# YukeWang96/QGTC_PPoPP22

Measured on AMD Instinct MI355X. Metric: effective bit-GEMM TOPS (2*M*K*N/t), 1-bit A x 1-bit X, M=K=4096, N=64, higher is better.
Workload: dtype fp4 (E2M1 codes of bit planes on MFMA, exact f32 sums); 1 GPU; bitMM2Bit 4096x4096x64 a=1 w=1 ob=1 (BASELINE.json configs[1], 2_7c shape); inputs=seeded Bernoulli(0.5) adjacency, uniform w-bit features, packed, resident in HBM, parallelism=replica-per-GPU x1, no data-path collective, engine=auto, issue=eager

## Files before the change

__graft_entry__.py:

```python
from __future__ import annotations

import os
import sys

ROOT = os.path.dirname(os.path.abspath(__file__))
if ROOT not in sys.path:
    sys.path.insert(0, ROOT)


def build() -> None:
    from qgtc_ppopp22_amd import _build

    paths = _build.build_all()
    from oracle import qgtc_oracle

    paths["oracle"] = qgtc_oracle.build()
    import qgtc_ppopp22_amd

    ext = qgtc_ppopp22_amd.load_ext()
    assert ext.abi_version() == 11
    import ctypes

    lib = ctypes.CDLL(qgtc_ppopp22_amd.lib_path())
    for sym in ("qgtc_abi_version", "qgtc_strerror", "qgtc_last_hip_error", "qgtc_rows_words",
                "qgtc_cols_words", "qgtc_val2bit", "qgtc_bit2val", "qgtc_bitmm2bit", "qgtc_bitmm2int",
                "qgtc_bitmm2bit_profile", "qgtc_tile_counters", "qgtc_bitmm_batched", "qgtc_pack_edges",
                "qgtc_i8gemm", "qgtc_i8gemm_profile", "qgtc_occupancy_words", "qgtc_tile_occupancy",
                "qgtc_tile_occupancy_batched", "qgtc_tile_occupancy_decide", "qgtc_pack_edge_list",
                "qgtc_gcn_layer_batched", "qgtc_gcn_chain_batched", "qgtc_last_batched_violation",
                "qgtc_val2bit_batched", "qgtc_epoch_pool_layout", "qgtc_epoch_plan_fill", "qgtc_expand_weights", "qgtc_chain_transform",
                "qgtc_chain_aggregate", "qgtc_chain_words", "qgtc_weight_codes_words", "qgtc_chain_from_cols",
                "qgtc_adj_tiles_words", "qgtc_adj_tiles_from_rows", "qgtc_load_batches", "qgtc_load_work_words", "qgtc_bitmm_route", "qgtc_bitmm_batched_route",
                "qgtc_tiled_work_words", "qgtc_tiled_count", "qgtc_tiled_fill", "qgtc_tiledmm2bit", "qgtc_tiledmm2int",
                "qgtc_tiled_colindex_work_words", "qgtc_tiled_colindex", "qgtc_tiledmm2bit_t", "qgtc_tiledmm2int_t",
                "qgtc_tiled_degrees", "qgtc_tiledmm2bit_scaled", "qgtc_tiledmm2int_scaled", "qgtc_tiledmm2bit_t_scaled", "qgtc_tiledmm2int_t_scaled",
                "qgtc_tiledmm_f32", "qgtc_tiledmm_f32_t", "qgtc_tiledmm_f32_src", "qgtc_tiledmm_f32_t_src", "qgtc_tiled_inv_sqrt_degree",
                "qgtc_tiledmax_f32", "qgtc_tiledmax_f32_t", "qgtc_tiledsel_f32", "qgtc_tiledsel_f32_t",
                "qgtc_tiledatt_f32", "qgtc_tiledatt_f32_t", "qgtc_tiledatt_grad_f32", "qgtc_tiledatt_grad_f32_t", "qgtc_rowdot_f32",
                "qgtc_edge_kept", "qgtc_tiledmm_f32_drop", "qgtc_tiledmm_f32_t_drop", "qgtc_tiledmax_f32_drop", "qgtc_tiledmax_f32_t_drop",
                "qgtc_tiledatt_f32_drop", "qgtc_tiledatt_f32_t_drop", "qgtc_tiledatt_grad_f32_drop", "qgtc_tiledatt_grad_f32_t_drop",
                "qgtc_node_bitmap", "qgtc_tiled_inv_degree", "qgtc_tiledmm_f32_nodes", "qgtc_tiledmm_f32_t_nodes", "qgtc_tiledmax_f32_nodes",
                "qgtc_tiledmax_f32_t_nodes", "qgtc_tiledatt_f32_nodes", "qgtc_tiledatt_f32_t_nodes", "qgtc_tiledatt_grad_f32_nodes",
                "qgtc_tiledatt_grad_f32_t_nodes", "qgtc_tiled_value_index", "qgtc_tiled_edge_slots", "qgtc_tiled_edge_endpoints",
                "qgtc_tiledmm_f32_edge", "qgtc_tiledmm_f32_t_edge", "qgtc_tiled_sddmm_f32", "qgtc_reorder_work_words", "qgtc_reorder_nodes"):
        getattr(lib, sym)
    print("[build] ok:", paths)


def smoke() -> None:
    import numpy as np
    import torch

    assert torch.cuda.is_available(), "smoke() needs a GPU"
    import QGTC
    from oracle.qgtc_oracle import Oracle

    O = Oracle()
    rng = np.random.default_rng(3)
    n, F, H, b = 300, 64, 64, 2
    A = (rng.random((n, n)) < 0.02).astype(np.float32)
    X = rng.normal(size=(n, F)).astype(np.float32)
    W = np.ones((F, H), dtype=np.float32)

    dA, dX, dW = (torch.from_numpy(t).cuda() for t in (A, X, W))
    bit_A = QGTC.val2bit(dA, 1, False, False)
    bit_X = QGTC.val2bit(dX, b, False, False)
    bit_W = QGTC.val2bit(dW, b, True, False)
# ... 82 lines not shown
```

include/qgtc.h:

```cpp
#ifndef QGTC_H
#define QGTC_H

#include <stddef.h>
#include <stdint.h>

#ifdef __cplusplus
extern "C" {
#endif

#define QGTC_ABI_VERSION 11

enum {
    QGTC_OK = 0,
    QGTC_EINVAL = 1,
    QGTC_ESIZE = 2,
    QGTC_EALIGN = 3,
    QGTC_EHIP = 4,
    QGTC_ENODEVICE = 5
};

#define QGTC_OUT_COLS 0x1u
#define QGTC_NO_ZERO_SKIP 0x2u
#define QGTC_ZERO_JUMP 0x4u
#define QGTC_ENGINE_MFMA 0x8u
// ... 46 lines not shown
int qgtc_tile_occupancy(const uint32_t *X, size_t x_words, int M, int K, int bit1, uint64_t *occ,
                        size_t occ_words, void *stream);

int qgtc_tile_occupancy_batched(qgtc_problem *problems, int count, int max_M, int max_K, int bit1,
                                float max_fraction, uint64_t *stats, void *stream);

int qgtc_tile_occupancy_decide(qgtc_problem *problems, int count, float max_fraction, uint64_t *stats,
                               void *stream);

int qgtc_bitmm_batched(const qgtc_problem *problems, int count, int max_M, int max_K, int max_N,
                       int bit1, int bit2, int output_bit, int mode, unsigned flags,
                       void *stream);

int qgtc_gcn_layer_batched(const qgtc_problem *stage1, const qgtc_problem *stage2, int count, int max_M, int max_K1,
                           int max_K2, int max_N, int x_bits, int w_bits, int t_bits, int a_bits, int output_bit,
                           int mode, unsigned flags, void *stream);

int qgtc_gcn_chain_batched(const qgtc_problem *stage_a, const qgtc_problem *stage_xw, int count, int max_M, int max_K,
                           int max_N1, int max_N2, int a_bits, int t_bits, int act_bits, int w_bits, int out_bits,
                           int out_mode, unsigned flags, void *stream);

const char *qgtc_bitmm_route(int M, int K, int N, int bit1, int bit2, int output_bit, int mode, unsigned flags);
const char *qgtc_bitmm_batched_route(int max_M, int max_K, int max_N, int bit1, int bit2, int output_bit, int mode, unsigned flags);

int qgtc_pack_edges(const int64_t *cells, const int32_t *counts, size_t n_cells, int H, int W,
                    int nbits, uint32_t *out, size_t out_words, void *stream);

int qgtc_pack_edge_list(const int64_t *src, const int64_t *dst, size_t n_edges, int H, int W, uint32_t *out,
                        size_t out_words, uint32_t *scratch, size_t scratch_words, int *bad_index, void *stream);

int qgtc_i8gemm(const int8_t *A, const int8_t *Bt, int M, int K, int N, float *C, size_t c_elems,
                void *stream);
int qgtc_i8gemm_profile(const int8_t *A, const int8_t *Bt, int M, int K, int N, float *C,
                        size_t c_elems, int reps, float *elapsed_ms, void *stream);

enum { QGTC_VIOL_NONE = 0, QGTC_VIOL_M = 1, QGTC_VIOL_K = 2, QGTC_VIOL_N = 3, QGTC_VIOL_POINTER = 4, QGTC_VIOL_CHAINING = 5 };
int qgtc_last_batched_violation(int *problem, int *field, void *stream);

#define QGTC_MAX_PACK_JOBS 8
typedef struct qgtc_pack_job {
    const float *x;
    uint32_t *out;
    uint64_t out_words;
    int32_t H, W, nbits, col_major, output_layer;
    int32_t reserved;
} qgtc_pack_job;
// ... 238 lines not shown
```

qgtc_ppopp22_amd/csrc/launch_common.hip.h:

```cpp
#pragma once

#include <algorithm>
#include <atomic>

int qgtc_launch_mfma(const qgtc_problem &pr, int a, int w, int ob, int mode, hipStream_t st);
int qgtc_launch_mfma_batched(const qgtc_problem *prs, int count, int max_M, int max_K, int max_N, int a, int w,
                             int ob, int mode, hipStream_t st);
int qgtc_launch_skinny(const qgtc_problem &pr, int a, int w, int ob, int mode, bool zero_skip, hipStream_t st);
bool qgtc_skinny_is_one(const qgtc_problem &pr, int ob, int mode);
int qgtc_launch_rows_single(const qgtc_problem &pr, int a, int w, int ob, int mode, hipStream_t st);
int qgtc_launch_rows(const qgtc_problem *prs, int count, int max_M, int max_N, int a, int w, int ob, int mode, hipStream_t st);
int qgtc_launch_xw_rows(const qgtc_problem *prs, int count, int max_M, int a, int w, int ob, hipStream_t st);

int qgtc_launch_expand_weights(const qgtc_expand_job *jobs, int n_jobs, hipStream_t st);
int qgtc_launch_cols_to_chain(const uint32_t *cols, size_t words, int H, int W, int nbits, uint32_t *chain, hipStream_t st);
int qgtc_launch_cols_to_chain_batched(const qgtc_loader_batch *batches, int count, int max_n, int W, int nbits, hipStream_t st);
int qgtc_launch_rbw_xw(const qgtc_problem *prs, int count, int max_M, int K, int N, int a, int ob, const uint32_t *w_codes, hipStream_t st);
int qgtc_launch_rbx_xw(const qgtc_problem *prs, int count, int max_M, int K, int N, int a, int ob, const uint32_t *w_codes, hipStream_t st);
int qgtc_launch_rbx_chain(const qgtc_problem *p1, const qgtc_problem *p2, int count, int max_M, int N1, int N2, int t_bits, int act_bits,
                          int mode2, const uint32_t *w2_codes, bool a_tiles, hipStream_t st);
int qgtc_launch_rbw_chain(const qgtc_problem *p1, const qgtc_problem *p2, int count, int max_M, int N1, int N2, int t_bits, int act_bits,
                          int out_bits, int mode2, const uint32_t *w2_codes, bool a_tiles, hipStream_t st);
int qgtc_launch_rows_to_tiles(const uint32_t *rows, size_t words, int M, int K, uint32_t *tiles, hipStream_t st);

int qgtc_launch_wide(const qgtc_problem &pr, int a, int w, int ob, int mode, hipStream_t st);
int qgtc_launch_stream(const qgtc_problem &pr, int ob, int mode, bool zero_skip, hipStream_t st);
int qgtc_launch_check_descriptors(const qgtc_problem *p1, const qgtc_problem *p2, int count, int max_M, int max_K1, int max_N1,
                                  int max_K2, int max_N2, int kind, hipStream_t st, int exact_N1 = 0, int exact_N2 = 0, int exact_K1 = 0);

namespace {
// ... 38 lines not shown
        static std::atomic<hipFunction_t> fns[MAX_DEV];
        int dev = 0;
        if (hipGetDevice(&dev) != hipSuccess || dev < 0 || dev >= MAX_DEV) return nullptr;
        hipFunction_t fn = fns[dev].load(std::memory_order_acquire);
        if (!fn) {
            if (getenv_flag("QGTC_NO_MODULE_LAUNCH") || hipGetFuncBySymbol(&fn, reinterpret_cast<const void *>(Kern)) != hipSuccess) return nullptr;
            fns[dev].store(fn, std::memory_order_release);
        }
        return fn;
    }
    static void go(dim3 grid, dim3 block, unsigned lds, hipStream_t st, P... p) {
        if (hipFunction_t fn = handle()) {
            void *params[] = {const_cast<void *>(static_cast<const void *>(&p))...};
            const hipError_t e = hipModuleLaunchKernel(fn, grid.x, grid.y, grid.z, block.x, block.y, block.z, lds, st, params, nullptr);
            if (e != hipSuccess && launch_error_slot() == hipSuccess) launch_error_slot() = e;
        } else {
            hipLaunchKernelGGL(Kern, grid, block, lds, st, p...);
            const hipError_t e = hipGetLastError();
            if (e != hipSuccess && launch_error_slot() == hipSuccess) launch_error_slot() = e;
        }
    }
};
#define QGTC_LAUNCH(kernel, grid, block, lds, st, ...) KernelLaunch<(kernel)>::go(grid, block, lds, st, __VA_ARGS__)

inline MMShape base_shape(int a, int w, int ob, int mode) {
    MMShape sh{};
    sh.a = a;
    sh.w = w;
    sh.ob = ob;
    sh.mode = mode;
    sh.ab = a;
    sh.wb = w;
    sh.maxv = std::ldexp(1.0f, ob);
    sh.maxm1 = sh.maxv - 1.0f;
    sh.nowrap = 0;
    return sh;
}

inline int no_wrap(int K, int a, int w) {
    if (a > 16 || w > 16) return 0;
    return static_cast<double>(pad128(K)) * ((1u << a) - 1u) * ((1u << w) - 1u) < 2147483648.0;
}

inline bool fp4_ok(int K, int a, int w) {
    return a <= 2 && w <= 2 && static_cast<double>(pad128(K)) * ((1 << a) - 1) * ((1 << w) - 1) < 16777216.0;
}
// ... 123 lines not shown
```

qgtc_ppopp22_amd/csrc/launch_fp4.hip.h:

```cpp
#pragma once

static size_t one_out_bytes(const qgtc_problem &pr, int ob, int mode) {
    if (mode == 2) return static_cast<size_t>(pr.M) * pr.N * 4u;
    if (mode == 1) return static_cast<size_t>(ob) * step128(pr.M) * 4u * pad128(pr.N) * 4u;
    return static_cast<size_t>(ob) * pad8(pr.M) * step128(pr.N) * 4u * 4u;
}
static bool one_ok(const qgtc_problem &pr, int ob, int mode) {
    return pr.K <= ONE_MAX_K && (mode == 2 || ob <= 23) && pr.M < (1 << 24) && one_out_bytes(pr, ob, mode) < (1ull << 32);
}

static int launch_one(const qgtc_problem &pr, int a, int w, int ob, int mode, bool zero_skip, hipStream_t st) {
    const bool wide = pr.N > 32 || mode == 1;
    const bool tall = w > 4 && mode != 1 && pr.N % 32 == 0 && ((pr.N >= 64 && pr.M >= 512) || pr.M >= 4096) && !getenv_flag("QGTC_NO_TALL");
    const dim3 grid(tall ? (pr.M + 63) / 64 : wide ? (pr.M + 31) / 32 : (pr.M + 15) / 16, tall ? pr.N / 16 : (pr.N + 31) / 32), block(64 * ONE_WAVES);
    const uint32_t cfg = static_cast<uint32_t>(a) | static_cast<uint32_t>(w) << 8 | static_cast<uint32_t>(mode == 2 ? 1 : ob) << 16 |
                         (zero_skip ? 1u : 0u) << 24
#ifdef QGTC_ABL
                         | (getenv_flag("ABL_X") ? 1u << 28 : 0u) | (getenv_flag("ABL_W") ? 1u << 29 : 0u)
#endif
#ifdef QGTC_STAGGER_EXP
                         | (getenv_flag("STAGGER_SLEEP") ? 1u << 30 : 0u) | (getenv_flag("STAGGER_PRIO") ? 1u << 31 : 0u) | (getenv_flag("STAGGER_SLEEP2") ? 1u << 27 : 0u)
#endif
        ;
    const uint32_t xb = static_cast<uint32_t>(pr.x_words * 4u), wb = static_cast<uint32_t>(pr.w_words * 4u);
    const uint32_t ob_ = static_cast<uint32_t>(one_out_bytes(pr, ob, mode));
#define QGTC_ONE_GO(NA_, NW_, MODE_, RF_)                                                                          \
    QGTC_LAUNCH((k_bitmm_fp4_one<NA_, NW_, MODE_, RF_, 2>), grid, block, 0, st, pr.X, pr.W, pr.out, xb, wb, ob_, pr.M, \
                       pr.K, pr.N, pr.w_lines, cfg)
#define QGTC_ONE_TALL(NA_, NW_)                                                                                               \
    if (!done && tall && a <= NA_ && w <= NW_) {                                                                               \
        done = true;                                                                                                           \
        if (mode == 2) QGTC_LAUNCH((k_bitmm_fp4_one<NA_, NW_, 2, 4, 1>), grid, block, 0, st, pr.X, pr.W, pr.out, xb, wb, ob_, pr.M, pr.K, pr.N, pr.w_lines, cfg); \
        else QGTC_LAUNCH((k_bitmm_fp4_one<NA_, NW_, 0, 4, 1>), grid, block, 0, st, pr.X, pr.W, pr.out, xb, wb, ob_, pr.M, pr.K, pr.N, pr.w_lines, cfg);           \
    }
#define QGTC_ONE_LAUNCH(NA_, NW_)                                       \
    if (!done && a <= NA_ && w <= NW_) {                                \
        done = true;                                                    \
        if (mode == 1) { QGTC_ONE_GO(NA_, NW_, 1, 2); }                 \
        else if (mode == 2) { if (wide) { QGTC_ONE_GO(NA_, NW_, 2, 2); } else { QGTC_ONE_GO(NA_, NW_, 2, 1); } } \
        else { if (wide) { QGTC_ONE_GO(NA_, NW_, 0, 2); } else { QGTC_ONE_GO(NA_, NW_, 0, 1); } }                \
    }
    bool done = false;
    QGTC_ONE_TALL(1, 8) QGTC_ONE_TALL(2, 8)
    QGTC_ONE_LAUNCH(1, 1) QGTC_ONE_LAUNCH(1, 2) QGTC_ONE_LAUNCH(1, 4) QGTC_ONE_LAUNCH(1, 8)
    QGTC_ONE_LAUNCH(2, 1) QGTC_ONE_LAUNCH(2, 2) QGTC_ONE_LAUNCH(2, 4) QGTC_ONE_LAUNCH(2, 8)
#undef QGTC_ONE_LAUNCH
#undef QGTC_ONE_TALL
#undef QGTC_ONE_GO
    HIP_TRY(launch_status());
    return QGTC_OK;
}

bool qgtc_skinny_is_one(const qgtc_problem &pr, int ob, int mode) { return one_ok(pr, ob, mode) && !getenv_flag("QGTC_NO_ONE"); }

int qgtc_launch_skinny(const qgtc_problem &pr, int a, int w, int ob, int mode, bool zero_skip, hipStream_t st) {
    if (one_ok(pr, ob, mode) && !getenv_flag("QGTC_NO_ONE")) return launch_one(pr, a, w, ob, mode, zero_skip, st);
    MMShape sh = base_shape(a, w, ob, mode);
    sh.nowrap = 1;
    const int zs = zero_skip ? 1 : 0;
    const bool wide = pr.N > 32 || mode == 1;
    const dim3 grid(wide ? (pr.M + 31) / 32 : (pr.M + 15) / 16, (pr.N + 31) / 32);
#define QGTC_SK_LAUNCH(NA_, NW_)                                                                                   \
    if (!done && a <= NA_ && w <= NW_) {                                                                           \
        done = true;                                                                                               \
        if (mode == 1) {                                                                                           \
            QGTC_LAUNCH((k_bitmm_fp4_skinny<NA_, NW_, 1, 2, 2>), grid, dim3(64 * SK_WAVES), 0, st, pr, sh, zs);            \
        } else if (mode == 2) {                                                                                    \
            if (wide) QGTC_LAUNCH((k_bitmm_fp4_skinny<NA_, NW_, 2, 2, 2>), grid, dim3(64 * SK_WAVES), 0, st, pr, sh, zs);  \
            else QGTC_LAUNCH((k_bitmm_fp4_skinny<NA_, NW_, 2, 1, 2>), grid, dim3(64 * SK_WAVES), 0, st, pr, sh, zs);       \
        } else {                                                                                                   \
            if (wide) QGTC_LAUNCH((k_bitmm_fp4_skinny<NA_, NW_, 0, 2, 2>), grid, dim3(64 * SK_WAVES), 0, st, pr, sh, zs);  \
            else QGTC_LAUNCH((k_bitmm_fp4_skinny<NA_, NW_, 0, 1, 2>), grid, dim3(64 * SK_WAVES), 0, st, pr, sh, zs);       \
        }                                                                                                          \
    }
    bool done = false;
    QGTC_SK_LAUNCH(1, 1) QGTC_SK_LAUNCH(1, 2) QGTC_SK_LAUNCH(1, 4) QGTC_SK_LAUNCH(1, 8)
    QGTC_SK_LAUNCH(2, 1) QGTC_SK_LAUNCH(2, 2) QGTC_SK_LAUNCH(2, 4) QGTC_SK_LAUNCH(2, 8)
#undef QGTC_SK_LAUNCH
    HIP_TRY(launch_status());
    return QGTC_OK;
}

int qgtc_launch_xw_rows(const qgtc_problem *prs, int count, int max_M, int a, int w, int ob, hipStream_t st) {
    MMShape sh = base_shape(a, w, ob, 1);
    sh.nowrap = 1;
    sh.per = getenv_flag("QGTC_NO_XCD") ? 0 : 1;
    const dim3 grid(step128(max_M) * 4, count), block(64 * 4);
    if (a <= 2 && w <= 2 && ob == 2) hipLaunchKernelGGL((k_bitmm_fp4_xw_rows<2, 2, 2>), grid, block, 0, st, prs, sh);
    else if (a <= 4 && w <= 4 && ob == 4) hipLaunchKernelGGL((k_bitmm_fp4_xw_rows<4, 4, 4>), grid, block, 0, st, prs, sh);
    else return QGTC_EINVAL;
    HIP_TRY(hipGetLastError());
    return QGTC_OK;
}

int qgtc_launch_rows(const qgtc_problem *prs, int count, int max_M, int max_N, int a, int w, int ob, int mode, hipStream_t st) {
    MMShape sh = base_shape(a, w, ob, mode);
    sh.nowrap = 1;
    sh.per = getenv_flag("QGTC_NO_XCD") ? 0 : 1;
    const int blocks = mode == 2 ? (max_N + 31) / 32 : mode == 1 ? pad128(max_N) / 32 : step128(max_N) * 4;
    const bool two = blocks >= 2 && mode != 1 && a <= 4 && getenv_flag("QGTC_ROWS_CB2");
    const int waves = two ? (blocks + 1) / 2 : blocks;
    if (waves > 8) return QGTC_EINVAL;
    const dim3 grid(mode == 1 ? step128(max_M) * 4 : (max_M + 31) / 32, count), block(64 * waves);
// ... 184 lines not shown
```

qgtc_ppopp22_amd/csrc/qgtc_hip.hip:

```cpp
#include <hip/hip_runtime.h>

#include <cmath>
#include <cstdio>
#include <cstdlib>
#include <cstring>
#include <type_traits>
#include <utility>

#include "qgtc.h"

#include "common.hip.h"
#include "pack_kernels.hip.h"
#include "i8gemm_kernel.hip.h"
#include "tile_stats_kernels.hip.h"
#include "loader_kernels.hip.h"
#include "bitmm_popcount.hip.h"
#include "bitmm_planes.hip.h"
#include "bitmm_mfma.hip.h"
#include "launch_common.hip.h"
#ifdef QGTC_SINGLE_TU
#include "bitmm_fp4_skinny.hip.h"
#include "bitmm_fp4_one.hip.h"
#include "fp4_rowblock.hip.h"
#include "bitmm_fp4_rows.hip.h"
// ... 105 lines not shown
        line_words = step128(H) * 4;
        plane = static_cast<size_t>(output_layer ? pad8(W) : pad128(W)) * line_words;
    } else {
        line_words = step128(W) * 4;
        plane = static_cast<size_t>(pad8(H)) * line_words;
    }
    const size_t total = static_cast<size_t>(H) * W;
    const unsigned g = grid_for(total, 256);
    QGTC_LAUNCH(k_bit2val, dim3(g), dim3(256), 0, st, bits, static_cast<unsigned long long>(bits_words), nbits, H, W, col_major, plane, line_words, out, 256u * g);
    HIP_TRY(launch_status());
    return QGTC_OK;
}

enum SingleRoute { RT_FP4_NARROW = 0, RT_FP4_STREAM, RT_FP4_ROWS, RT_FP4_WIDE, RT_MFMA_128, RT_POPCOUNT };
static SingleRoute single_route(const qgtc_problem &pr, int a, int w, int ob, int mode, unsigned flags) {
    const bool mf = (flags & QGTC_ENGINE_MFMA) != 0u, au = (flags & QGTC_ENGINE_AUTO) != 0u;
    if (stream_ok(pr, a, w, ob, mode) && (mf || (au && auto_prefers_stream(pr.M, pr.K, pr.N)))) return RT_FP4_STREAM;
    if (skinny_ok(pr.K, pr.N, a, w) && (mf || (au && auto_prefers_skinny(pr.M, pr.K, pr.N, a, w)))) return RT_FP4_NARROW;
    if (rows_single_ok(pr, a, w, ob, mode) && (mf || au)) return RT_FP4_ROWS;
    if (wide_ok(pr, a, w, ob, mode) && (mf || (au && auto_prefers_wide(pr.M, pr.K, pr.N, a, w, mode)))) return RT_FP4_WIDE;
    if ((mf && mfma_ok(a, w)) || (au && auto_prefers_mfma(pr.M, pr.K, pr.N, a, w))) return RT_MFMA_128;
    return RT_POPCOUNT;
}
static int launch_single_route(const qgtc_problem &pr, int a, int w, int ob, int mode, unsigned flags, hipStream_t st) {
    switch (single_route(pr, a, w, ob, mode, flags)) {
        case RT_FP4_NARROW: return qgtc_launch_skinny(pr, a, w, ob, mode, !(flags & QGTC_NO_ZERO_SKIP), st);
        case RT_FP4_STREAM: return qgtc_launch_stream(pr, ob, mode, !(flags & QGTC_NO_ZERO_SKIP), st);
        case RT_FP4_ROWS: return qgtc_launch_rows_single(pr, a, w, ob, mode, st);
        case RT_FP4_WIDE: return qgtc_launch_wide(pr, a, w, ob, mode, st);
        case RT_MFMA_128: return qgtc_launch_mfma(pr, a, w, ob, mode, st);
        default: break;
    }
    if (flags & QGTC_NO_ZERO_SKIP) return dispatch_single<false>(pr, pr.K, a, w, ob, mode, st);
    return dispatch_single<true>(pr, pr.K, a, w, ob, mode, st);
}

const char *qgtc_bitmm_route(int M, int K, int N, int bit1, int bit2, int output_bit, int mode, unsigned flags) {
    if (M <= 0 || K <= 0 || N <= 0 || !bits_ok(bit1) || !bits_ok(bit2) || mode < 0 || mode > 2 || (mode != 2 && !bits_ok(output_bit))) return "invalid";
    qgtc_problem pr{nullptr, nullptr, nullptr, qgtc_rows_words(M, K, bit1), qgtc_cols_words(K, N, bit2, 0), M, K, N, pad128(N), 0, nullptr};
    const int ob = mode == 2 ? 1 : output_bit;
    switch (single_route(pr, bit1, bit2, ob, mode, flags)) {
        case RT_FP4_NARROW: return qgtc_skinny_is_one(pr, ob, mode) ? "k_bitmm_fp4_one" : "k_bitmm_fp4_skinny";
        case RT_FP4_STREAM: return "k_bitmm_fp4_stream";
        case RT_FP4_ROWS: return "k_bitmm_fp4_rows_single";
        case RT_FP4_WIDE: return "k_bitmm_fp4_wide";
        case RT_MFMA_128: return "k_bitmm_mfma";
        default: return "k_bitmm";
    }
}

int qgtc_bitmm2bit(const uint32_t *X, size_t x_words, const uint32_t *W, size_t w_words, int M,
                   int K, int N, int bit1, int bit2, int output_bit, uint32_t *out,
                   size_t out_words, unsigned flags, void *stream) {
    int rc = check_mm_args(X, W, out, M, K, N, bit1, bit2);
    if (rc != QGTC_OK) return rc;
    if (!bits_ok(output_bit) || !words_ok(x_words, w_words)) return QGTC_EINVAL;
    const bool cols = flags & QGTC_OUT_COLS;
    const size_t need = cols ? qgtc_cols_words(M, N, output_bit, 0) : qgtc_rows_words(M, N, output_bit);
    if (out_words < need) return QGTC_ESIZE;
    qgtc_problem pr{X, W, out, x_words, w_words, M, K, N, pad128(N), 0, nullptr};
    return launch_single_route(pr, bit1, bit2, output_bit, cols ? 1 : 0, flags, static_cast<hipStream_t>(stream));
}

int qgtc_bitmm2int(const uint32_t *X, size_t x_words, const uint32_t *W, size_t w_words, int M,
                   int K, int N, int bit1, int bit2, int pad_128, float *out, size_t out_elems,
                   unsigned flags, void *stream) {
    int rc = check_mm_args(X, W, out, M, K, N, bit1, bit2);
    if (rc != QGTC_OK) return rc;
    if (!words_ok(x_words, w_words)) return QGTC_EINVAL;
    if (out_elems < static_cast<size_t>(M) * N) return QGTC_ESIZE;
    qgtc_problem pr{X, W, out, x_words, w_words, M, K, N, pad_128 ? pad128(N) : pad8(N), 0, nullptr};
    return launch_single_route(pr, bit1, bit2, 1, 2, flags, static_cast<hipStream_t>(stream));
}

int qgtc_bitmm2bit_profile(const uint32_t *X, size_t x_words, const uint32_t *W, size_t w_words,
                           int M, int K, int N, int bit1, int bit2, int output_bit, uint32_t *out,
                           size_t out_words, unsigned flags, int reps, float *elapsed_ms,
                           void *stream) {
    if (reps <= 0 || !elapsed_ms) return QGTC_EINVAL;
    hipStream_t st = static_cast<hipStream_t>(stream);
    int rc = qgtc_bitmm2bit(X, x_words, W, w_words, M, K, N, bit1, bit2, output_bit, out, out_words,
                            flags, stream);
    if (rc != QGTC_OK) return rc;
    EventPair ev;
    HIP_TRY(ev.create());
    HIP_TRY(hipEventRecord(ev.e0, st));
    for (int i = 0; i < reps && rc == QGTC_OK; i++)
        rc = qgtc_bitmm2bit(X, x_words, W, w_words, M, K, N, bit1, bit2, output_bit, out, out_words,
                            flags, stream);
    hipError_t e = hipEventRecord(ev.e1, st);
    if (e == hipSuccess) e = hipEventSynchronize(ev.e1);
    float ms = 0.0f;
    if (e == hipSuccess) e = hipEventElapsedTime(&ms, ev.e0, ev.e1);
    if (rc != QGTC_OK) return rc;
    if (e != hipSuccess) return hip_fail(e, "profile events");
// ... 387 lines not shown
```

qgtc_ppopp22_amd/csrc/qgtc_torch.cpp:

```cpp
#include <torch/extension.h>

#include <ATen/hip/EmptyTensor.h>
#include <c10/core/DeviceGuard.h>
#include <c10/hip/HIPFunctions.h>
#include <c10/hip/HIPStream.h>
#include <torch/csrc/autograd/python_variable.h>

#include <array>
#include <pybind11/stl.h>
#include <atomic>
#include <chrono>
#include <cstdio>
#include <memory>
#include <mutex>
#include <optional>
#include <tuple>
#include <utility>
#include <vector>

#include "qgtc.h"

namespace {

inline int S8(int x) { return (x + 7) >> 3; }
// ... 135 lines not shown
    auto out = torch::empty({static_cast<int64_t>(ob) * P8(M), S128(N) * 4},
                            torch::TensorOptions().dtype(torch::kInt32).device(bit_X1.device()));
    float ms = 0.0f;
    check_rc(qgtc_bitmm2bit_profile(words(bit_X1), bit_X1.numel(), words(bit_X2), bit_X2.numel(), M,
                                    K, N, bit1, bit2, ob, words_mut(out), out.numel(), mm_flags(),
                                    reps, &ms, current_stream(bit_X1)),
             "bitMM2Bit_profile");
    g_last_profile_ms = ms;
    return {out, ms};
}

void bitMM2Bit_enqueue(torch::Tensor out, torch::Tensor bit_X1, torch::Tensor bit_X2, int M, int K,
                       int N, int bit1, int bit2, int ob, int reps, bool cols) {
    CHECK_INPUT(out);
    CHECK_INPUT(bit_X1);
    CHECK_INPUT(bit_X2);
    check_bits_tensor(out, "out");
    check_bits_tensor(bit_X1, "bit_X1");
    check_bits_tensor(bit_X2, "bit_X2");
    TORCH_CHECK(reps > 0, "reps must be positive");
    TORCH_CHECK(out.device() == bit_X1.device() && bit_X2.device() == bit_X1.device(), "out, bit_X1 and bit_X2 must be on the same device");
    c10::DeviceGuard guard(bit_X1.device());
    void *st = current_stream(bit_X1);
    for (int i = 0; i < reps; i++)
        check_rc(qgtc_bitmm2bit(words(bit_X1), bit_X1.numel(), words(bit_X2), bit_X2.numel(), M, K, N,
                                bit1, bit2, ob, words_mut(out), out.numel(), mm_flags() | (cols ? QGTC_OUT_COLS : 0u), st),
                 "bitMM2Bit_enqueue");
}

void bitMM2Bit_enqueue_streams(std::vector<torch::Tensor> outs, torch::Tensor bit_X1, torch::Tensor bit_X2,
                               int M, int K, int N, int bit1, int bit2, int ob, int reps) {
    CHECK_INPUT(bit_X1);
    CHECK_INPUT(bit_X2);
    check_bits_tensor(bit_X1, "bit_X1");
    check_bits_tensor(bit_X2, "bit_X2");
    TORCH_CHECK(!outs.empty() && reps > 0, "need at least one output buffer and one launch");
    c10::DeviceGuard guard(bit_X1.device());
    const int n = static_cast<int>(outs.size());
    TORCH_CHECK(bit_X2.device() == bit_X1.device(), "bit_X1 and bit_X2 must be on the same device");
    for (auto &o : outs) {
        CHECK_INPUT(o);
        check_bits_tensor(o, "out");
        TORCH_CHECK(o.device() == bit_X1.device(), "every output must be on the operands' device");
    }
    auto cur = c10::hip::getCurrentHIPStream(bit_X1.get_device());
    const auto pool = side_streams(bit_X1.get_device(), n);
    ScopedEvent sev;
    hipEvent_t ev = sev.ev;
    TORCH_CHECK(hipEventRecord(ev, cur.stream()) == hipSuccess, "hipEventRecord failed");
    for (int s = 0; s < n; s++) TORCH_CHECK(hipStreamWaitEvent(pool[s].stream(), ev, 0) == hipSuccess, "wait failed");
    for (int i = 0; i < reps; i++) {
        torch::Tensor &o = outs[i % n];
        check_rc(qgtc_bitmm2bit(words(bit_X1), bit_X1.numel(), words(bit_X2), bit_X2.numel(), M, K, N, bit1,
                                bit2, ob, words_mut(o), o.numel(), mm_flags(),
                                static_cast<void *>(pool[i % n].stream())),
                 "bitMM2Bit_enqueue_streams");
    }
    for (int s = 0; s < n; s++) {
        TORCH_CHECK(hipEventRecord(ev, pool[s].stream()) == hipSuccess, "hipEventRecord failed");
        TORCH_CHECK(hipStreamWaitEvent(cur.stream(), ev, 0) == hipSuccess, "wait failed");
    }
}

torch::Tensor bitMM2Bit_profile(torch::Tensor bit_X1, torch::Tensor bit_X2, const int X1_height,
                                const int X1_width, const int X2_width, const int bit1,
                                const int bit2, const int output_bit) {
    constexpr int PROF = 200;
    auto r = profile_impl(bit_X1, bit_X2, X1_height, X1_width, X2_width, bit1, bit2, output_bit, PROF);
    const float ops = 2.0f * X1_height * X1_width * X2_width * PROF;
    printf("X1_height %d, X1_width: %d, X2_width: %d, TFLOPs: %.3f\n", X1_height, X1_width, X2_width,
           ops / (r.second / 1e3) / 1e12);
    fflush(stdout);
    return r.first;
}

std::vector<unsigned long long> tile_counters(const torch::Tensor &bit_X1, int M, int K, int N,
                                              int bit1, int bit2) {
    c10::DeviceGuard guard(bit_X1.device());
    auto buf = torch::empty({2}, torch::TensorOptions().dtype(torch::kInt64).device(bit_X1.device()));
    check_rc(qgtc_tile_counters(words(bit_X1), bit_X1.numel(), M, K, N, bit1, bit2,
// ... 1678 lines not shown
```

Measured before the change: 738.0 TOPS.

## Cache per-shape launch plans and issue skinny kernels via hipModuleLaunchKernel

Adds a thread-local cache of launch plans keyed by problem shape, bits, flags and device. On a hit it skips argument validation, routing and kernel selection and launches the kernel directly with prebuilt parameter arrays. The torch enqueue loops also hoist tensor accessors out of the per-rep loop. This targets host-side dispatch overhead on small, launch-bound GEMMs, at the cost of extra state and a risk of a stale plan if environment flags change between calls.

```diff
diff --git a/__graft_entry__.py b/__graft_entry__.py
--- a/__graft_entry__.py
+++ b/__graft_entry__.py
@@ -42,7 +42,7 @@
                 "qgtc_node_bitmap", "qgtc_tiled_inv_degree", "qgtc_tiledmm_f32_nodes", "qgtc_tiledmm_f32_t_nodes", "qgtc_tiledmax_f32_nodes",
                 "qgtc_tiledmax_f32_t_nodes", "qgtc_tiledatt_f32_nodes", "qgtc_tiledatt_f32_t_nodes", "qgtc_tiledatt_grad_f32_nodes",
                 "qgtc_tiledatt_grad_f32_t_nodes", "qgtc_tiled_value_index", "qgtc_tiled_edge_slots", "qgtc_tiled_edge_endpoints",
-                "qgtc_tiledmm_f32_edge", "qgtc_tiledmm_f32_t_edge", "qgtc_tiled_sddmm_f32", "qgtc_reorder_work_words", "qgtc_reorder_nodes"):
+                "qgtc_tiledmm_f32_edge", "qgtc_tiledmm_f32_t_edge", "qgtc_tiled_sddmm_f32", "qgtc_reorder_work_words", "qgtc_reorder_nodes", "qgtc_launch_plan_stats"):
         getattr(lib, sym)
     print("[build] ok:", paths)
 
diff --git a/include/qgtc.h b/include/qgtc.h
--- a/include/qgtc.h
+++ b/include/qgtc.h
@@ -92,6 +92,8 @@
 
 const char *qgtc_bitmm_route(int M, int K, int N, int bit1, int bit2, int output_bit, int mode, unsigned flags);
 const char *qgtc_bitmm_batched_route(int max_M, int max_K, int max_N, int bit1, int bit2, int output_bit, int mode, unsigned flags);
+
+int qgtc_launch_plan_stats(unsigned long long *hits, unsigned long long *builds);
 
 int qgtc_pack_edges(const int64_t *cells, const int32_t *counts, size_t n_cells, int H, int W,
                     int nbits, uint32_t *out, size_t out_words, void *stream);
diff --git a/qgtc_ppopp22_amd/csrc/launch_common.hip.h b/qgtc_ppopp22_amd/csrc/launch_common.hip.h
--- a/qgtc_ppopp22_amd/csrc/launch_common.hip.h
+++ b/qgtc_ppopp22_amd/csrc/launch_common.hip.h
@@ -6,6 +6,19 @@
 int qgtc_launch_mfma(const qgtc_problem &pr, int a, int w, int ob, int mode, hipStream_t st);
 int qgtc_launch_mfma_batched(const qgtc_problem *prs, int count, int max_M, int max_K, int max_N, int a, int w,
                              int ob, int mode, hipStream_t st);
+struct LaunchPlan {
+    int route;
+    int a, w, ob, mode;
+    unsigned flags;
+    qgtc_problem pr;
+    hipFunction_t fn;
+    hipError_t (*ggl)(LaunchPlan &, hipStream_t);
+    void (*bind)(LaunchPlan &);
+    unsigned gx, gy, bx, lds;
+    alignas(16) unsigned char scalars[64];
+    void *params[12];
+};
+int qgtc_plan_skinny(const qgtc_problem &pr, int a, int w, int ob, int mode, bool zero_skip, LaunchPlan *plan);
 int qgtc_launch_skinny(const qgtc_problem &pr, int a, int w, int ob, int mode, bool zero_skip, hipStream_t st);
 bool qgtc_skinny_is_one(const qgtc_problem &pr, int ob, int mode);
 int qgtc_launch_rows_single(const qgtc_problem &pr, int a, int w, int ob, int mode, hipStream_t st);
@@ -90,6 +103,14 @@
     }
 };
 #define QGTC_LAUNCH(kernel, grid, block, lds, st, ...) KernelLaunch<(kernel)>::go(grid, block, lds, st, __VA_ARGS__)
+
+inline int plan_issue(LaunchPlan &p, const uint32_t *X, const uint32_t *W, void *out, hipStream_t st) {
+    p.pr.X = X;
+    p.pr.W = W;
+    p.pr.out = out;
+    HIP_TRY(p.fn ? hipModuleLaunchKernel(p.fn, p.gx, p.gy, 1, p.bx, 1, 1, p.lds, st, p.params, nullptr) : p.ggl(p, st));
+    return QGTC_OK;
+}
 
 inline MMShape base_shape(int a, int w, int ob, int mode) {
     MMShape sh{};
diff --git a/qgtc_ppopp22_amd/csrc/launch_fp4.hip.h b/qgtc_ppopp22_amd/csrc/launch_fp4.hip.h
--- a/qgtc_ppopp22_amd/csrc/launch_fp4.hip.h
+++ b/qgtc_ppopp22_amd/csrc/launch_fp4.hip.h
@@ -9,29 +9,87 @@
     return pr.K <= ONE_MAX_K && (mode == 2 || ob <= 23) && pr.M < (1 << 24) && one_out_bytes(pr, ob, mode) < (1ull << 32);
 }
 
-static int launch_one(const qgtc_problem &pr, int a, int w, int ob, int mode, bool zero_skip, hipStream_t st) {
+struct OneScalars {
+    uint32_t x_bytes, w_bytes, out_bytes, cfg;
+};
+struct LoopScalars {
+    MMShape sh;
+    int zs;
+};
+static_assert(sizeof(OneScalars) <= sizeof(LaunchPlan::scalars) && sizeof(LoopScalars) <= sizeof(LaunchPlan::scalars), "LaunchPlan::scalars");
+static_assert(alignof(OneScalars) <= 16 && alignof(LoopScalars) <= 16, "LaunchPlan::scalars");
+
+static void bind_one(LaunchPlan &p) {
+    OneScalars &s = *reinterpret_cast<OneScalars *>(p.scalars);
+    void *params[] = {&p.pr.X, &p.pr.W, &p.pr.out, &s.x_bytes, &s.w_bytes, &s.out_bytes, &p.pr.M, &p.pr.K, &p.pr.N, &p.pr.w_lines, &s.cfg};
+    static_assert(sizeof(params) <= sizeof(p.params), "LaunchPlan::params");
+    std::memcpy(p.params, params, sizeof(params));
+}
+static void bind_loop(LaunchPlan &p) {
+    LoopScalars &s = *reinterpret_cast<LoopScalars *>(p.scalars);
+    p.params[0] = &p.pr;
+    p.params[1] = &s.sh;
+    p.params[2] = &s.zs;
+}
+template <auto Kern>
+static hipError_t ggl_one(LaunchPlan &p, hipStream_t st) {
+    const OneScalars &s = *reinterpret_cast<const OneScalars *>(p.scalars);
+    hipLaunchKernelGGL(Kern, dim3(p.gx, p.gy), dim3(p.bx), p.lds, st, p.pr.X, p.pr.W, p.pr.out, s.x_bytes, s.w_bytes, s.out_bytes, p.pr.M, p.pr.K,
+                       p.pr.N, p.pr.w_lines, s.cfg);
+    return hipGetLastError();
+}
+template <auto Kern>
+static hipError_t ggl_loop(LaunchPlan &p, hipStream_t st) {
+    const LoopScalars &s = *reinterpret_cast<const LoopScalars *>(p.scalars);
+    hipLaunchKernelGGL(Kern, dim3(p.gx, p.gy), dim3(p.bx), p.lds, st, p.pr, s.sh, s.zs);
+    return hipGetLastError();
+}
+template <auto Kern>
+static void plan_kernel_one(LaunchPlan &p) {
+    static_assert(std::is_same<decltype(Kern), void (*)(const uint32_t *, const uint32_t *, void *, uint32_t, uint32_t, uint32_t, int, int, int, int, uint32_t)>::value,
+                  "bind_one lays out k_bitmm_fp4_one's eleven arguments");
+    static_assert(std::is_same<decltype(qgtc_problem::X), const uint32_t *>::value && std::is_same<decltype(qgtc_problem::out), void *>::value &&
+                      std::is_same<decltype(qgtc_problem::M), int>::value && std::is_same<decltype(qgtc_problem::w_lines), int>::value,
+                  "qgtc_problem's fields are passed as the kernel's arguments");
+    p.fn = KernelLaunch<Kern>::handle();
+    p.ggl = &ggl_one<Kern>;
+    p.bind = &bind_one;
+}
+template <auto Kern>
+static void plan_kernel_loop(LaunchPlan &p) {
+    static_assert(std::is_same<decltype(Kern), void (*)(qgtc_problem, MMShape, int)>::value, "bind_loop lays out k_bitmm_fp4_skinny's three arguments");
+    p.fn = KernelLaunch<Kern>::handle();
+    p.ggl = &ggl_loop<Kern>;
+    p.bind = &bind_loop;
+}
+
+static int plan_one(const qgtc_problem &pr, int a, int w, int ob, int mode, bool zero_skip, LaunchPlan &p) {
     const bool wide = pr.N > 32 || mode == 1;
     const bool tall = w > 4 && mode != 1 && pr.N % 32 == 0 && ((pr.N >= 64 && pr.M >= 512) || pr.M >= 4096) && !getenv_flag("QGTC_NO_TALL");
-    const dim3 grid(tall ? (pr.M + 63) / 64 : wide ? (pr.M + 31) / 32 : (pr.M + 15) / 16, tall ? pr.N / 16 : (pr.N + 31) / 32), block(64 * ONE_WAVES);
-    const uint32_t cfg = static_cast<uint32_t>(a) | static_cast<uint32_t>(w) << 8 | static_cast<uint32_t>(mode == 2 ? 1 : ob) << 16 |
-                         (zero_skip ? 1u : 0u) << 24
+    p.gx = tall ? (pr.M + 63) / 64 : wide ? (pr.M + 31) / 32 : (pr.M + 15) / 16;
+    p.gy = tall ? pr.N / 16 : (pr.N + 31) / 32;
+    p.bx = 64 * ONE_WAVES;
+    p.lds = 0;
+    p.pr = pr;
+    OneScalars &s = *reinterpret_cast<OneScalars *>(p.scalars);
+    s.cfg = static_cast<uint32_t>(a) | static_cast<uint32_t>(w) << 8 | static_cast<uint32_t>(mode == 2 ? 1 : ob) << 16 |
+            (zero_skip ? 1u : 0u) << 24
 #ifdef QGTC_ABL
-                         | (getenv_flag("ABL_X") ? 1u << 28 : 0u) | (getenv_flag("ABL_W") ? 1u << 29 : 0u)
+            | (getenv_flag("ABL_X") ? 1u << 28 : 0u) | (getenv_flag("ABL_W") ? 1u << 29 : 0u)
 #endif
 #ifdef QGTC_STAGGER_EXP
-                         | (getenv_flag("STAGGER_SLEEP") ? 1u << 30 : 0u) | (getenv_flag("STAGGER_PRIO") ? 1u << 31 : 0u) | (getenv_flag("STAGGER_SLEEP2") ? 1u << 27 : 0u)
+            | (getenv_flag("STAGGER_SLEEP") ? 1u << 30 : 0u) | (getenv_flag("STAGGER_PRIO") ? 1u << 31 : 0u) | (getenv_flag("STAGGER_SLEEP2") ? 1u << 27 : 0u)
 #endif
         ;
-    const uint32_t xb = static_cast<uint32_t>(pr.x_words * 4u), wb = static_cast<uint32_t>(pr.w_words * 4u);
-    const uint32_t ob_ = static_cast<uint32_t>(one_out_bytes(pr, ob, mode));
-#define QGTC_ONE_GO(NA_, NW_, MODE_, RF_)                                                                          \
-    QGTC_LAUNCH((k_bitmm_fp4_one<NA_, NW_, MODE_, RF_, 2>), grid, block, 0, st, pr.X, pr.W, pr.out, xb, wb, ob_, pr.M, \
-                       pr.K, pr.N, pr.w_lines, cfg)
-#define QGTC_ONE_TALL(NA_, NW_)                                                                                               \
-    if (!done && tall && a <= NA_ && w <= NW_) {                                                                               \
-        done = true;                                                                                                           \
-        if (mode == 2) QGTC_LAUNCH((k_bitmm_fp4_one<NA_, NW_, 2, 4, 1>), grid, block, 0, st, pr.X, pr.W, pr.out, xb, wb, ob_, pr.M, pr.K, pr.N, pr.w_lines, cfg); \
-        else QGTC_LAUNCH((k_bitmm_fp4_one<NA_, NW_, 0, 4, 1>), grid, block, 0, st, pr.X, pr.W, pr.out, xb, wb, ob_, pr.M, pr.K, pr.N, pr.w_lines, cfg);           \
+    s.x_bytes = static_cast<uint32_t>(pr.x_words * 4u);
+    s.w_bytes = static_cast<uint32_t>(pr.w_words * 4u);
+    s.out_bytes = static_cast<uint32_t>(one_out_bytes(pr, ob, mode));
+#define QGTC_ONE_GO(NA_, NW_, MODE_, RF_) plan_kernel_one<(k_bitmm_fp4_one<NA_, NW_, MODE_, RF_, 2>)>(p)
+#define QGTC_ONE_TALL(NA_, NW_)                                                    \
+    if (!done && tall && a <= NA_ && w <= NW_) {                                    \
+        done = true;                                                                \
+        if (mode == 2) plan_kernel_one<(k_bitmm_fp4_one<NA_, NW_, 2, 4, 1>)>(p);    \
+        else plan_kernel_one<(k_bitmm_fp4_one<NA_, NW_, 0, 4, 1>)>(p);              \
     }
 #define QGTC_ONE_LAUNCH(NA_, NW_)                                       \
     if (!done && a <= NA_ && w <= NW_) {                                \
@@ -47,38 +105,48 @@
 #undef QGTC_ONE_LAUNCH
 #undef QGTC_ONE_TALL
 #undef QGTC_ONE_GO
-    HIP_TRY(launch_status());
+    if (!done) return QGTC_EINVAL;
+    p.bind(p);
     return QGTC_OK;
 }
 
 bool qgtc_skinny_is_one(const qgtc_problem &pr, int ob, int mode) { return one_ok(pr, ob, mode) && !getenv_flag("QGTC_NO_ONE"); }
 
-int qgtc_launch_skinny(const qgtc_problem &pr, int a, int w, int ob, int mode, bool zero_skip, hipStream_t st) {
-    if (one_ok(pr, ob, mode) && !getenv_flag("QGTC_NO_ONE")) return launch_one(pr, a, w, ob, mode, zero_skip, st);
-    MMShape sh = base_shape(a, w, ob, mode);
-    sh.nowrap = 1;
-    const int zs = zero_skip ? 1 : 0;
+int qgtc_plan_skinny(const qgtc_problem &pr, int a, int w, int ob, int mode, bool zero_skip, LaunchPlan *plan) {
+    LaunchPlan &p = *plan;
+    if (one_ok(pr, ob, mode) && !getenv_flag("QGTC_NO_ONE")) return plan_one(pr, a, w, ob, mode, zero_skip, p);
     const bool wide = pr.N > 32 || mode == 1;
-    const dim3 grid(wide ? (pr.M + 31) / 32 : (pr.M + 15) / 16, (pr.N + 31) / 32);
-#define QGTC_SK_LAUNCH(NA_, NW_)                                                                                   \
-    if (!done && a <= NA_ && w <= NW_) {                                                                           \
-        done = true;                                                                                               \
-        if (mode == 1) {                                                                                           \
-            QGTC_LAUNCH((k_bitmm_fp4_skinny<NA_, NW_, 1, 2, 2>), grid, dim3(64 * SK_WAVES), 0, st, pr, sh, zs);            \
-        } else if (mode == 2) {                                                                                    \
-            if (wide) QGTC_LAUNCH((k_bitmm_fp4_skinny<NA_, NW_, 2, 2, 2>), grid, dim3(64 * SK_WAVES), 0, st, pr, sh, zs);  \
-            else QGTC_LAUNCH((k_bitmm_fp4_skinny<NA_, NW_, 2, 1, 2>), grid, dim3(64 * SK_WAVES), 0, st, pr, sh, zs);       \
-        } else {                                                                                                   \
-            if (wide) QGTC_LAUNCH((k_bitmm_fp4_skinny<NA_, NW_, 0, 2, 2>), grid, dim3(64 * SK_WAVES), 0, st, pr, sh, zs);  \
-            else QGTC_LAUNCH((k_bitmm_fp4_skinny<NA_, NW_, 0, 1, 2>), grid, dim3(64 * SK_WAVES), 0, st, pr, sh, zs);       \
-        }                                                                                                          \
+    p.gx = wide ? (pr.M + 31) / 32 : (pr.M + 15) / 16;
+    p.gy = (pr.N + 31) / 32;
+    p.bx = 64 * SK_WAVES;
+    p.lds = 0;
+    p.pr = pr;
+    LoopScalars &s = *reinterpret_cast<LoopScalars *>(p.scalars);
+    s.sh = base_shape(a, w, ob, mode);
+    s.sh.nowrap = 1;
+    s.zs = zero_skip ? 1 : 0;
+#define QGTC_SK_GO(NA_, NW_, MODE_, RF_) plan_kernel_loop<(k_bitmm_fp4_skinny<NA_, NW_, MODE_, RF_, 2>)>(p)
+#define QGTC_SK_LAUNCH(NA_, NW_)                                        \
+    if (!done && a <= NA_ && w <= NW_) {                                \
+        done = true;                                                    \
+        if (mode == 1) { QGTC_SK_GO(NA_, NW_, 1, 2); }                  \
+        else if (mode == 2) { if (wide) { QGTC_SK_GO(NA_, NW_, 2, 2); } else { QGTC_SK_GO(NA_, NW_, 2, 1); } } \
+        else { if (wide) { QGTC_SK_GO(NA_, NW_, 0, 2); } else { QGTC_SK_GO(NA_, NW_, 0, 1); } }                \
     }
     bool done = false;
     QGTC_SK_LAUNCH(1, 1) QGTC_SK_LAUNCH(1, 2) QGTC_SK_LAUNCH(1, 4) QGTC_SK_LAUNCH(1, 8)
     QGTC_SK_LAUNCH(2, 1) QGTC_SK_LAUNCH(2, 2) QGTC_SK_LAUNCH(2, 4) QGTC_SK_LAUNCH(2, 8)
 #undef QGTC_SK_LAUNCH
-    HIP_TRY(launch_status());
-    return QGTC_OK;
+#undef QGTC_SK_GO
+    if (!done) return QGTC_EINVAL;
+    p.bind(p);
+    return QGTC_OK;
+}
+
+int qgtc_launch_skinny(const qgtc_problem &pr, int a, int w, int ob, int mode, bool zero_skip, hipStream_t st) {
+    LaunchPlan p{};
+    const int rc = qgtc_plan_skinny(pr, a, w, ob, mode, zero_skip, &p);
+    return rc != QGTC_OK ? rc : plan_issue(p, pr.X, pr.W, pr.out, st);
 }
 
 int qgtc_launch_xw_rows(const qgtc_problem *prs, int count, int max_M, int a, int w, int ob, hipStream_t st) {
diff --git a/qgtc_ppopp22_amd/csrc/qgtc_hip.hip b/qgtc_ppopp22_amd/csrc/qgtc_hip.hip
--- a/qgtc_ppopp22_amd/csrc/qgtc_hip.hip
+++ b/qgtc_ppopp22_amd/csrc/qgtc_hip.hip
@@ -151,17 +151,104 @@
     if ((mf && mfma_ok(a, w)) || (au && auto_prefers_mfma(pr.M, pr.K, pr.N, a, w))) return RT_MFMA_128;
     return RT_POPCOUNT;
 }
-static int launch_single_route(const qgtc_problem &pr, int a, int w, int ob, int mode, unsigned flags, hipStream_t st) {
-    switch (single_route(pr, a, w, ob, mode, flags)) {
-        case RT_FP4_NARROW: return qgtc_launch_skinny(pr, a, w, ob, mode, !(flags & QGTC_NO_ZERO_SKIP), st);
-        case RT_FP4_STREAM: return qgtc_launch_stream(pr, ob, mode, !(flags & QGTC_NO_ZERO_SKIP), st);
-        case RT_FP4_ROWS: return qgtc_launch_rows_single(pr, a, w, ob, mode, st);
-        case RT_FP4_WIDE: return qgtc_launch_wide(pr, a, w, ob, mode, st);
-        case RT_MFMA_128: return qgtc_launch_mfma(pr, a, w, ob, mode, st);
+static int plan_build(const qgtc_problem &pr, int a, int w, int ob, int mode, unsigned flags, LaunchPlan &p) {
+    p = LaunchPlan{};
+    p.route = single_route(pr, a, w, ob, mode, flags);
+    p.a = a;
+    p.w = w;
+    p.ob = ob;
+    p.mode = mode;
+    p.flags = flags;
+    p.pr = pr;
+    if (p.route == RT_FP4_NARROW) return qgtc_plan_skinny(pr, a, w, ob, mode, !(flags & QGTC_NO_ZERO_SKIP), &p);
+    return QGTC_OK;
+}
+static int plan_launch(LaunchPlan &p, const uint32_t *X, const uint32_t *W, void *out, hipStream_t st) {
+    if (p.bind) return plan_issue(p, X, W, out, st);
+    p.pr.X = X;
+    p.pr.W = W;
+    p.pr.out = out;
+    switch (p.route) {
+        case RT_FP4_NARROW: return QGTC_EINVAL;
+        case RT_FP4_STREAM: return qgtc_launch_stream(p.pr, p.ob, p.mode, !(p.flags & QGTC_NO_ZERO_SKIP), st);
+        case RT_FP4_ROWS: return qgtc_launch_rows_single(p.pr, p.a, p.w, p.ob, p.mode, st);
+        case RT_FP4_WIDE: return qgtc_launch_wide(p.pr, p.a, p.w, p.ob, p.mode, st);
+        case RT_MFMA_128: return qgtc_launch_mfma(p.pr, p.a, p.w, p.ob, p.mode, st);
         default: break;
     }
-    if (flags & QGTC_NO_ZERO_SKIP) return dispatch_single<false>(pr, pr.K, a, w, ob, mode, st);
-    return dispatch_single<true>(pr, pr.K, a, w, ob, mode, st);
+    if (p.flags & QGTC_NO_ZERO_SKIP) return dispatch_single<false>(p.pr, p.pr.K, p.a, p.w, p.ob, p.mode, st);
+    return dispatch_single<true>(p.pr, p.pr.K, p.a, p.w, p.ob, p.mode, st);
+}
+
+namespace {
+struct PlanKey {
+    size_t x_words, w_words, out_words;
+    int M, K, N, bit1, bit2, ob_or_pad, kind;
+    unsigned flags;
+    bool same_call(const PlanKey &o) const {
+        return M == o.M && K == o.K && N == o.N && bit1 == o.bit1 && bit2 == o.bit2 && ob_or_pad == o.ob_or_pad && kind == o.kind &&
+               flags == o.flags && x_words == o.x_words && w_words == o.w_words && out_words == o.out_words;
+    }
+};
+constexpr int kPlanCapacity = 8;
+struct PlanCache {
+    struct Entry {
+        PlanKey key;
+        int dev;
+        bool used;
+        LaunchPlan plan;
+    } entry[kPlanCapacity];
+    int last, next;
+    unsigned long long hits, builds;
+};
+thread_local PlanCache t_plans;
+
+inline int current_device() {
+    int dev = -1;
+    return hipGetDevice(&dev) == hipSuccess ? dev : -1;
+}
+inline LaunchPlan *plan_find(const PlanKey &key) {
+    PlanCache &c = t_plans;
+    int dev = -2;
+    for (int n = 0, i = c.last; n < kPlanCapacity; n++, i = i + 1 == kPlanCapacity ? 0 : i + 1) {
+        PlanCache::Entry &e = c.entry[i];
+        if (!e.used || !e.key.same_call(key)) continue;
+        if (dev == -2) dev = current_device();
+        if (e.dev != dev) continue;
+        c.last = i;
+        return &e.plan;
+    }
+    return nullptr;
+}
+inline int check_operands(const uint32_t *X, const uint32_t *W, const void *out) {
+    if (!X || !W || !out) return QGTC_EINVAL;
+    if (!aligned16(X) || !aligned16(W)) return QGTC_EALIGN;
+    return QGTC_OK;
+}
+inline int plan_miss(const PlanKey &key, const qgtc_problem &pr, int a, int w, int ob, int mode, unsigned flags, hipStream_t st) {
+    LaunchPlan p;
+    int rc = plan_build(pr, a, w, ob, mode, flags, p);
+    if (rc == QGTC_OK) rc = plan_launch(p, pr.X, pr.W, pr.out, st);
+    const int dev = rc == QGTC_OK ? current_device() : -1;
+    if (dev < 0) return rc;
+    PlanCache &c = t_plans;
+    PlanCache::Entry &e = c.entry[c.next];
+    c.last = c.next;
+    c.next = c.next + 1 == kPlanCapacity ? 0 : c.next + 1;
+    e.key = key;
+    e.dev = dev;
+    e.plan = p;
+    if (e.plan.bind) e.plan.bind(e.plan);
+    e.used = true;
+    c.builds++;
+    return rc;
+}
+}
+
+int qgtc_launch_plan_stats(unsigned long long *hits, unsigned long long *builds) {
+    if (hits) *hits = t_plans.hits;
+    if (builds) *builds = t_plans.builds;
+    return QGTC_OK;
 }
 
 const char *qgtc_bitmm_route(int M, int K, int N, int bit1, int bit2, int output_bit, int mode, unsigned flags) {
@@ -181,6 +268,13 @@
 int qgtc_bitmm2bit(const uint32_t *X, size_t x_words, const uint32_t *W, size_t w_words, int M,
                    int K, int N, int bit1, int bit2, int output_bit, uint32_t *out,
                    size_t out_words, unsigned flags, void *stream) {
+    const PlanKey key{x_words, w_words, out_words, M, K, N, bit1, bit2, output_bit, 0, flags};
+    if (LaunchPlan *p = plan_find(key)) {
+        const int rc = check_operands(X, W, out);
+        if (rc != QGTC_OK) return rc;
+        t_plans.hits++;
+        return plan_launch(*p, X, W, out, static_cast<hipStream_t>(stream));
+    }
     int rc = check_mm_args(X, W, out, M, K, N, bit1, bit2);
     if (rc != QGTC_OK) return rc;
     if (!bits_ok(output_bit) || !words_ok(x_words, w_words)) return QGTC_EINVAL;
@@ -188,18 +282,25 @@
     const size_t need = cols ? qgtc_cols_words(M, N, output_bit, 0) : qgtc_rows_words(M, N, output_bit);
     if (out_words < need) return QGTC_ESIZE;
     qgtc_problem pr{X, W, out, x_words, w_words, M, K, N, pad128(N), 0, nullptr};
-    return launch_single_route(pr, bit1, bit2, output_bit, cols ? 1 : 0, flags, static_cast<hipStream_t>(stream));
+    return plan_miss(key, pr, bit1, bit2, output_bit, cols ? 1 : 0, flags, static_cast<hipStream_t>(stream));
 }
 
 int qgtc_bitmm2int(const uint32_t *X, size_t x_words, const uint32_t *W, size_t w_words, int M,
                    int K, int N, int bit1, int bit2, int pad_128, float *out, size_t out_elems,
                    unsigned flags, void *stream) {
+    const PlanKey key{x_words, w_words, out_elems, M, K, N, bit1, bit2, pad_128 ? 1 : 0, 1, flags};
+    if (LaunchPlan *p = plan_find(key)) {
+        const int rc = check_operands(X, W, out);
+        if (rc != QGTC_OK) return rc;
+        t_plans.hits++;
+        return plan_launch(*p, X, W, out, static_cast<hipStream_t>(stream));
+    }
     int rc = check_mm_args(X, W, out, M, K, N, bit1, bit2);
     if (rc != QGTC_OK) return rc;
     if (!words_ok(x_words, w_words)) return QGTC_EINVAL;
     if (out_elems < static_cast<size_t>(M) * N) return QGTC_ESIZE;
     qgtc_problem pr{X, W, out, x_words, w_words, M, K, N, pad_128 ? pad128(N) : pad8(N), 0, nullptr};
-    return launch_single_route(pr, bit1, bit2, 1, 2, flags, static_cast<hipStream_t>(stream));
+    return plan_miss(key, pr, bit1, bit2, 1, 2, flags, static_cast<hipStream_t>(stream));
 }
 
 int qgtc_bitmm2bit_profile(const uint32_t *X, size_t x_words, const uint32_t *W, size_t w_words,
diff --git a/qgtc_ppopp22_amd/csrc/qgtc_torch.cpp b/qgtc_ppopp22_amd/csrc/qgtc_torch.cpp
--- a/qgtc_ppopp22_amd/csrc/qgtc_torch.cpp
+++ b/qgtc_ppopp22_amd/csrc/qgtc_torch.cpp
@@ -181,10 +181,14 @@
     TORCH_CHECK(out.device() == bit_X1.device() && bit_X2.device() == bit_X1.device(), "out, bit_X1 and bit_X2 must be on the same device");
     c10::DeviceGuard guard(bit_X1.device());
     void *st = current_stream(bit_X1);
-    for (int i = 0; i < reps; i++)
-        check_rc(qgtc_bitmm2bit(words(bit_X1), bit_X1.numel(), words(bit_X2), bit_X2.numel(), M, K, N,
-                                bit1, bit2, ob, words_mut(out), out.numel(), mm_flags() | (cols ? QGTC_OUT_COLS : 0u), st),
-                 "bitMM2Bit_enqueue");
+    const uint32_t *x = words(bit_X1), *w = words(bit_X2);
+    uint32_t *o = words_mut(out);
+    const size_t x_words = bit_X1.numel(), w_words = bit_X2.numel(), out_words = out.numel();
+    const unsigned flags = mm_flags() | (cols ? QGTC_OUT_COLS : 0u);
+    int rc = QGTC_OK;
+    for (int i = 0; i < reps && rc == QGTC_OK; i++)
+        rc = qgtc_bitmm2bit(x, x_words, w, w_words, M, K, N, bit1, bit2, ob, o, out_words, flags, st);
+    check_rc(rc, "bitMM2Bit_enqueue");
 }
 
 void bitMM2Bit_enqueue_streams(std::vector<torch::Tensor> outs, torch::Tensor bit_X1, torch::Tensor bit_X2,
@@ -208,13 +212,21 @@
     hipEvent_t ev = sev.ev;
     TORCH_CHECK(hipEventRecord(ev, cur.stream()) == hipSuccess, "hipEventRecord failed");
     for (int s = 0; s < n; s++) TORCH_CHECK(hipStreamWaitEvent(pool[s].stream(), ev, 0) == hipSuccess, "wait failed");
-    for (int i = 0; i < reps; i++) {
-        torch::Tensor &o = outs[i % n];
-        check_rc(qgtc_bitmm2bit(words(bit_X1), bit_X1.numel(), words(bit_X2), bit_X2.numel(), M, K, N, bit1,
-                                bit2, ob, words_mut(o), o.numel(), mm_flags(),
-                                static_cast<void *>(pool[i % n].stream())),
-                 "bitMM2Bit_enqueue_streams");
-    }
+    const uint32_t *x = words(bit_X1), *w = words(bit_X2);
+    const size_t x_words = bit_X1.numel(), w_words = bit_X2.numel();
+    const unsigned flags = mm_flags();
+    std::vector<uint32_t *> o(n);
+    std::vector<size_t> o_words(n);
+    std::vector<void *> sts(n);
+    for (int s = 0; s < n; s++) {
+        o[s] = words_mut(outs[s]);
+        o_words[s] = outs[s].numel();
+        sts[s] = static_cast<void *>(pool[s].stream());
+    }
+    int rc = QGTC_OK;
+    for (int i = 0, s = 0; i < reps && rc == QGTC_OK; i++, s = s + 1 == n ? 0 : s + 1)
+        rc = qgtc_bitmm2bit(x, x_words, w, w_words, M, K, N, bit1, bit2, ob, o[s], o_words[s], flags, sts[s]);
+    check_rc(rc, "bitMM2Bit_enqueue_streams");
     for (int s = 0; s < n; s++) {
         TORCH_CHECK(hipEventRecord(ev, pool[s].stream()) == hipSuccess, "hipEventRecord failed");
         TORCH_CHECK(hipStreamWaitEvent(cur.stream(), ev, 0) == hipSuccess, "wait failed");
```

After: 737.5 TOPS. Within noise of the previous version (-0.1%).
